# youmi-zym/GO-SLAM

Measured on AMD Instinct MI355X. Metric: BA keyframes/s (6 x FactorGraph.update: reproject + corr lookup + GRU + 2 GN BA iters) on synthetic 640x480 RGB-D, higher is better.
Workload: dtype f32 (BA/geometry; fp64 solve), f16 (corr volume, GRU convs); 1 GPU; configs[1]-shaped frontend window: 60x80 maps (480x640 RGB-D), P=25 keyframes, E=75 edges, 6 updates/keyframe, iters=2, RGB-D depth prior, upsample on; parallelism=replicas x1 (tracking does not shard)

## Files before the change

### go_slam_amd/csrc/gru_gates.hip

```cpp
#include "common.h"

namespace {

typedef _Float16 half8 __attribute__((ext_vector_type(8)));

__device__ __forceinline__ float sigm(float x) { return gs_sigmoid(x); }

__global__ __launch_bounds__(256) void gru_gate_zr_kernel(const _Float16* __restrict__ zr_pre,
                                                          const float* __restrict__ bias,
                                                          const float* __restrict__ glo,
                                                          const _Float16* __restrict__ inp_pre,
                                                          _Float16* __restrict__ hx,
                                                          _Float16* __restrict__ z_out, int hw, int ldx,
                                                          size_t total ) {
  const size_t t = (size_t)blockIdx.x * 256 + threadIdx.x;
  if (t >= total) return;
  const int c8 = (int)(t & 15);
  const size_t pix = t >> 4;
  const int n = (int)(pix / hw);
  const half8 zp = *reinterpret_cast<const half8*>(zr_pre + pix * 256 + c8 * 8);
  const half8 rp = *reinterpret_cast<const half8*>(zr_pre + pix * 256 + 128 + c8 * 8);
  half8* hp = reinterpret_cast<half8*>(hx + pix * ldx + c8 * 8);
  const half8 net = *hp;
  half8 zi = {0, 0, 0, 0, 0, 0, 0, 0}, ri = zi;
  if (inp_pre) {
    zi = *reinterpret_cast<const half8*>(inp_pre + pix * 384 + c8 * 8);
    ri = *reinterpret_cast<const half8*>(inp_pre + pix * 384 + 128 + c8 * 8);
  }
  half8 zo, rn;
#pragma unroll
  for (int k = 0; k < 8; ++k) {
    const int c = c8 * 8 + k;
    const float z = sigm((float)zp[k] + (float)zi[k] + bias[c] + glo[(size_t)n * 256 + c]);
    const float r = sigm((float)rp[k] + (float)ri[k] + bias[128 + c] + glo[(size_t)n * 256 + 128 + c]);
    zo[k] = (_Float16)z;
    rn[k] = (_Float16)(r * (float)net[k]);
  }
  *reinterpret_cast<half8*>(z_out + pix * 128 + c8 * 8) = zo;
  *hp = rn;
}

__global__ __launch_bounds__(256) void gru_gate_q_kernel(const _Float16* __restrict__ q_pre,
                                                         const float* __restrict__ bias,
                                                         const float* __restrict__ glo,
                                                         const _Float16* __restrict__ inp_pre,
                                                         const _Float16* __restrict__ z, const _Float16* __restrict__ net,
                                                         _Float16* __restrict__ net_out, int hw, size_t total) {
  const size_t t = (size_t)blockIdx.x * 256 + threadIdx.x;
  if (t >= total) return;
  const int c8 = (int)(t & 15);
  const size_t pix = t >> 4;
  const int n = (int)(pix / hw);
  const size_t o = pix * 128 + c8 * 8;
  const half8 qp = *reinterpret_cast<const half8*>(q_pre + o);
  const half8 zz = *reinterpret_cast<const half8*>(z + o);
  const half8 nn = *reinterpret_cast<const half8*>(net + o);
  half8 qi = {0, 0, 0, 0, 0, 0, 0, 0};
  if (inp_pre) qi = *reinterpret_cast<const half8*>(inp_pre + pix * 384 + 256 + c8 * 8);
  half8 out;
#pragma unroll
  for (int k = 0; k < 8; ++k) {
    const int c = c8 * 8 + k;
    const float a = (float)qp[k] + (float)qi[k] + bias[c] + glo[(size_t)n * 128 + c];
    const float q = gs_tanh(a);
    const float zf = (float)zz[k];
    out[k] = (_Float16)((1.0f - zf) * (float)nn[k] + zf * q);
  }
  *reinterpret_cast<half8*>(net_out + o) = out;
}

}

extern "C" int gs_gru_gate_zr(const void* zr_pre, const float* bias_zr, const float* glo_zr, const void* inp_pre,
                              void* hx, void* z_out, int n, int hw, int ldx, gs_stream_t stream) {
  GS_REQUIRE(zr_pre && bias_zr && glo_zr && hx && z_out, "gru_gate_zr: null pointer");
  GS_REQUIRE(n >= 0 && hw > 0 && ldx >= 128 && ldx % 8 == 0, "gru_gate_zr: bad shape");
  if (n == 0) return GS_OK;
  const size_t total = (size_t)n * hw * 16;
  gru_gate_zr_kernel<<<(unsigned)((total + 255) / 256), 256, 0, (hipStream_t)stream>>>(
      (const _Float16*)zr_pre, bias_zr, glo_zr, (const _Float16*)inp_pre, (_Float16*)hx, (_Float16*)z_out, hw, ldx,
      total);
  GS_CHECK_LAUNCH("gru_gate_zr");
  return GS_OK;
}

extern "C" int gs_gru_gate_q(const void* q_pre, const float* bias_q, const float* glo_q, const void* inp_pre,
                             const void* z, const void* net, void* net_out, int n, int hw, gs_stream_t stream) {
  GS_REQUIRE(q_pre && bias_q && glo_q && z && net && net_out, "gru_gate_q: null pointer");
  GS_REQUIRE(n >= 0 && hw > 0, "gru_gate_q: bad shape");
  if (n == 0) return GS_OK;
  const size_t total = (size_t)n * hw * 16;
  gru_gate_q_kernel<<<(unsigned)((total + 255) / 256), 256, 0, (hipStream_t)stream>>>(
      (const _Float16*)q_pre, bias_q, glo_q, (const _Float16*)inp_pre, (const _Float16*)z, (const _Float16*)net,
      (_Float16*)net_out, hw, total);
  GS_CHECK_LAUNCH("gru_gate_q");
  return GS_OK;
}

namespace {
template <int ACT, bool BIAS>
__global__ __launch_bounds__(256) void bias_act_kernel(const _Float16* __restrict__ x, const float* __restrict__ bias,
                                                       _Float16* __restrict__ y, int c8n , int ldx, int ldy,
                                                       size_t total ) {
  const size_t t = (size_t)blockIdx.x * 256 + threadIdx.x;
  if (t >= total) return;
  const int c8 = (int)(t % c8n);
  const size_t row = t / c8n;
  half8 v = *reinterpret_cast<const half8*>(x + row * ldx + c8 * 8);
  if (BIAS || ACT) {
#pragma unroll
    for (int k = 0; k < 8; ++k) {
      float f = (float)v[k];
      if (BIAS) f += bias[c8 * 8 + k];
      if (ACT == 1) f = fmaxf(f, 0.0f);
      if (ACT == 2) f = sigm(f);
      v[k] = (_Float16)f;
    }
  }
  *reinterpret_cast<half8*>(y + row * ldy + c8 * 8) = v;
}

__global__ __launch_bounds__(256) void segment_mean_kernel(const _Float16* __restrict__ x, int ldx,
                                                           const float* __restrict__ in_bias, int in_relu,
                                                           const int* __restrict__ off, const int* __restrict__ edges,
                                                           _Float16* __restrict__ out, int hw, int c8n, size_t total) {
  const size_t t = (size_t)blockIdx.x * 256 + threadIdx.x;
  if (t >= total) return;
  const int c8 = (int)(t % c8n);
  const size_t sp = t / c8n;
  const int seg = (int)(sp / hw);
  const int p = (int)(sp - (size_t)seg * hw);
  const int b = off[seg], e = off[seg + 1];
  float bias[8], acc[8];
#pragma unroll
  for (int j = 0; j < 8; ++j) { bias[j] = in_bias ? in_bias[c8 * 8 + j] : 0.0f; acc[j] = 0.0f; }
  const bool touch = (in_bias != nullptr) || in_relu;
  for (int k0 = b; k0 < e; k0 += 4) {
    half8 v[4];
#pragma unroll
    for (int u = 0; u < 4; ++u) {
      const int k = min(k0 + u, e - 1);
      v[u] = *reinterpret_cast<const half8*>(x + ((size_t)edges[k] * hw + p) * ldx + c8 * 8);
    }
#pragma unroll
    for (int u = 0; u < 4; ++u) {
      if (k0 + u >= e) continue;
#pragma unroll
      for (int j = 0; j < 8; ++j) {
        float f = (float)v[u][j];
        if (touch) {
          f += bias[j];
          if (in_relu) f = fmaxf(f, 0.0f);
          f = (float)(_Float16)f;
        }
        acc[j] += f;
      }
    }
  }
  const float inv = e > b ? 1.0f / (float)(e - b) : 0.0f;
  half8 o;
#pragma unroll
  for (int j = 0; j < 8; ++j) o[j] = (_Float16)(acc[j] * inv);
  reinterpret_cast<half8*>(out)[t] = o;
}

__global__ __launch_bounds__(256) void glo_pool_kernel(const _Float16* __restrict__ w_pre, const float* __restrict__ bias,
                                                       const _Float16* __restrict__ net, float* __restrict__ partial,
                                                       int hw, int nchunk) {
  const int n = blockIdx.y, chunk = blockIdx.x;
  const int c8 = threadIdx.x & 15, lane = threadIdx.x >> 4;
  const int p0 = (int)((long)hw * chunk / nchunk), p1 = (int)((long)hw * (chunk + 1) / nchunk);
  float b[8], acc[8];
#pragma unroll
  for (int k = 0; k < 8; ++k) { b[k] = bias[c8 * 8 + k]; acc[k] = 0.0f; }
  for (int p = p0 + lane; p < p1; p += 16) {
    const size_t o = ((size_t)n * hw + p) * 128 + c8 * 8;
    const half8 w = *reinterpret_cast<const half8*>(w_pre + o);
    const half8 h = *reinterpret_cast<const half8*>(net + o);
#pragma unroll
    for (int k = 0; k < 8; ++k) {
      const _Float16 g = (_Float16)sigm((float)(_Float16)((float)w[k] + b[k]));
      acc[k] += (float)(_Float16)((float)g * (float)h[k]);
    }
  }
  __shared__ float red[16][129];
#pragma unroll
  for (int k = 0; k < 8; ++k) red[lane][c8 * 8 + k] = acc[k];
  __syncthreads();
  if (threadIdx.x < 128) {
    float s = 0.0f;
#pragma unroll
    for (int l = 0; l < 16; ++l) s += red[l][threadIdx.x];
    partial[((size_t)n * nchunk + chunk) * 128 + threadIdx.x] = s;
  }
}

typedef _Float16 half4g __attribute__((ext_vector_type(4)));
typedef float float16g __attribute__((ext_vector_type(16)));
__global__ __launch_bounds__(256) void glo_conv_pool_kernel(const _Float16* __restrict__ net, int ldx,
                                                            const _Float16* __restrict__ wpack,
                                                            const float* __restrict__ bias, float* __restrict__ partial,
                                                            int hw, int bpi, size_t nblk) {
  extern __shared__ _Float16 wl[];
  const int tid = threadIdx.x, lane = tid & 63, wv = tid >> 6;
  for (int i = tid; i < 4 * 8 * 64; i += 256) reinterpret_cast<half8*>(wl)[i] = reinterpret_cast<const half8*>(wpack)[i];
  __syncthreads();
  constexpr int TS = 72;
  _Float16* tile = wl + 4 * 8 * 512 + wv * 32 * TS;
  float* sbias = reinterpret_cast<float*>(wl + 4 * 8 * 512 + 4 * 32 * TS);
  if (tid < 128) sbias[tid] = bias[tid];
  __syncthreads();
  const int kh = 8 * (lane >> 5);
  const int piece = lane & 7;
  for (size_t blk = (size_t)blockIdx.x * 4 + wv; blk < nblk; blk += (size_t)gridDim.x * 4) {
    const size_t img = blk / bpi;
    const int b0 = (int)(blk - img * bpi) * 32;
    const int pin = b0 + (lane & 31);
    const _Float16* xr = net + (img * hw + (pin < hw ? pin : hw - 1)) * (size_t)ldx + kh;
    half8 bfr[8];
#pragma unroll
    for (int ks = 0; ks < 8; ++ks) bfr[ks] = *reinterpret_cast<const half8*>(xr + 16 * ks);
    half8 hrow[2][4];
#pragma unroll
    for (int it = 0; it < 4; ++it) {
      const int pxr = b0 + it * 8 + (lane >> 3);
      const _Float16* hr = net + (img * hw + (pxr < hw ? pxr : hw - 1)) * (size_t)ldx + piece * 8;
      hrow[0][it] = *reinterpret_cast<const half8*>(hr);
      hrow[1][it] = *reinterpret_cast<const half8*>(hr + 64);
    }
    float16g c[4];
#pragma unroll
    for (int q = 0; q < 4; ++q)
#pragma unroll
      for (int e = 0; e < 16; ++e) c[q][e] = 0.0f;
#pragma unroll
    for (int ks = 0; ks < 8; ++ks)
#pragma unroll
      for (int q = 0; q < 4; ++q) {
        const half8 a = *reinterpret_cast<const half8*>(wl + ((size_t)(q * 8 + ks) * 64 + lane) * 8);
        c[q] = __builtin_amdgcn_mfma_f32_32x32x16_f16(a, bfr[ks], c[q], 0, 0, 0);
      }
#pragma unroll
    for (int pr = 0; pr < 2; ++pr) {
#pragma unroll
      for (int qq = 0; qq < 2; ++qq)
#pragma unroll
        for (int g = 0; g < 4; ++g) {
          const int chl = qq * 32 + 8 * g + 4 * (lane >> 5);
          half4g o;
#pragma unroll
          for (int e = 0; e < 4; ++e)
            o[e] = (_Float16)sigm((float)(_Float16)(c[2 * pr + qq][4 * g + e] + sbias[pr * 64 + chl + e]));
          *reinterpret_cast<half4g*>(tile + (lane & 31) * TS + chl) = o;
        }
      __builtin_amdgcn_fence(__ATOMIC_RELEASE, "wavefront");
      __builtin_amdgcn_wave_barrier();
      __builtin_amdgcn_fence(__ATOMIC_ACQUIRE, "wavefront");
      float acc[8] = {0.f, 0.f, 0.f, 0.f, 0.f, 0.f, 0.f, 0.f};
#pragma unroll
      for (int it = 0; it < 4; ++it) {
        const int pxr = it * 8 + (lane >> 3);
        const half8 g8 = *reinterpret_cast<const half8*>(tile + pxr * TS + piece * 8);
        const half8 h8 = hrow[pr][it];
        const float live = (b0 + pxr < hw) ? 1.0f : 0.0f;
#pragma unroll
        for (int k = 0; k < 8; ++k) acc[k] += live * (float)(_Float16)((float)g8[k] * (float)h8[k]);
      }
#pragma unroll
      for (int k = 0; k < 8; ++k) {
        acc[k] += __shfl_xor(acc[k], 8);
        acc[k] += __shfl_xor(acc[k], 16);
        acc[k] += __shfl_xor(acc[k], 32);
      }
      if (lane < 8) {
        float* dst = partial + blk * 128 + pr * 64 + lane * 8;
        *reinterpret_cast<float4*>(dst) = make_float4(acc[0], acc[1], acc[2], acc[3]);
        *reinterpret_cast<float4*>(dst + 4) = make_float4(acc[4], acc[5], acc[6], acc[7]);
      }
      __builtin_amdgcn_fence(__ATOMIC_RELEASE, "wavefront");
      __builtin_amdgcn_wave_barrier();
    }
  }
}

__global__ __launch_bounds__(384) void glo_heads_kernel(const float* __restrict__ partial, int nchunk, float inv_hw,
                                                        const _Float16* __restrict__ wz, const _Float16* __restrict__ wr,
                                                        const _Float16* __restrict__ wq, const float* __restrict__ bz,
                                                        const float* __restrict__ br, const float* __restrict__ bq,
                                                        float* __restrict__ gzr, float* __restrict__ gq) {
  const int n = blockIdx.x, t = threadIdx.x;
  __shared__ float g[128];
  __shared__ float part3[3][128];
  {
    const int third = t >> 7, ch = t & 127;
    float s = 0.0f;
    for (int c0 = third; c0 < nchunk; c0 += 30) {
      float v[10];
#pragma unroll
      for (int u = 0; u < 10; ++u) {
        const int c = c0 + 3 * u;
        v[u] = c < nchunk ? partial[((size_t)n * nchunk + c) * 128 + ch] : 0.0f;
      }
#pragma unroll
      for (int u = 0; u < 10; ++u)
        if (c0 + 3 * u < nchunk) s += v[u];
    }
    part3[third][ch] = s;
  }
  __syncthreads();
  if (t < 128) g[t] = (float)(_Float16)(((part3[0][t] + part3[1][t]) + part3[2][t]) * inv_hw);
  __syncthreads();
  const int head = t >> 7, o = t & 127;
  const _Float16* w = (head == 0 ? wz : head == 1 ? wr : wq) + (size_t)o * 128;
  float s = (head == 0 ? bz : head == 1 ? br : bq)[o];
#pragma unroll 4
  for (int k8 = 0; k8 < 16; ++k8) {
    const half8 v = *reinterpret_cast<const half8*>(w + k8 * 8);
#pragma unroll
    for (int k = 0; k < 8; ++k) s = fmaf((float)v[k], g[k8 * 8 + k], s);
  }
  s = (float)(_Float16)s;
  if (head < 2) gzr[(size_t)n * 256 + head * 128 + o] = s;
  else gq[(size_t)n * 128 + o] = s;
}
}

extern "C" int gs_bias_act(const void* x, const float* bias, void* y, int rows, int channels, int x_stride,
                           int y_stride, int act, gs_stream_t stream) {
  GS_REQUIRE(x && y, "bias_act: null pointer");
  GS_REQUIRE(rows >= 0 && channels > 0 && channels % 8 == 0, "bias_act: channels must be a multiple of 8");
  GS_REQUIRE(x_stride >= channels && x_stride % 8 == 0, "bias_act: x_stride must be >= channels and a multiple of 8");
  GS_REQUIRE(y_stride >= channels && y_stride % 8 == 0, "bias_act: y_stride must be >= channels and a multiple of 8");
  GS_REQUIRE(act >= 0 && act <= 2, "bias_act: act in {0 none, 1 relu, 2 sigmoid}");
  if (rows == 0) return GS_OK;
  const size_t total = (size_t)rows * (channels / 8);
  const unsigned grid = (unsigned)((total + 255) / 256);
  hipStream_t st = (hipStream_t)stream;
  const _Float16* xi = (const _Float16*)x;
  _Float16* yo = (_Float16*)y;
  const int c8n = channels / 8;
#define GS_BA(A, B) bias_act_kernel<A, B><<<grid, 256, 0, st>>>(xi, bias, yo, c8n, x_stride, y_stride, total)
  if (bias) { if (act == 0) GS_BA(0, true); else if (act == 1) GS_BA(1, true); else GS_BA(2, true); }
  else      { if (act == 0) GS_BA(0, false); else if (act == 1) GS_BA(1, false); else GS_BA(2, false); }
#undef GS_BA
  GS_CHECK_LAUNCH("bias_act");
  return GS_OK;
}

extern "C" int gs_segment_mean(const void* x, int x_stride, const float* in_bias, int in_relu, const int* seg_offsets,
                               const int* seg_edges, void* out, int n_seg, int hw, int channels, gs_stream_t stream) {
  GS_REQUIRE(x && seg_offsets && seg_edges && out, "segment_mean: null pointer");
  GS_REQUIRE(n_seg >= 0 && hw > 0 && channels > 0 && channels % 8 == 0, "segment_mean: channels must be a multiple of 8");
  GS_REQUIRE(x_stride >= channels && x_stride % 8 == 0, "segment_mean: x_stride must be >= channels, multiple of 8");
  if (n_seg == 0) return GS_OK;
  const size_t total = (size_t)n_seg * hw * (channels / 8);
  segment_mean_kernel<<<(unsigned)((total + 255) / 256), 256, 0, (hipStream_t)stream>>>(
      (const _Float16*)x, x_stride, in_bias, in_relu, seg_offsets, seg_edges, (_Float16*)out, hw, channels / 8, total);
  GS_CHECK_LAUNCH("segment_mean");
  return GS_OK;
}

constexpr int GLO_CHUNKS = 32;
extern "C" size_t gs_gru_glo_workspace_bytes(int n) { return (size_t)(n > 0 ? n : 0) * GLO_CHUNKS * 128 * sizeof(float); }

extern "C" int gs_gru_glo(const void* w_pre, const float* w_bias, const void* net, const void* wz, const void* wr,
                          const void* wq, const float* bz, const float* br, const float* bq, float* gzr, float* gq,
                          int n, int hw, void* workspace, size_t workspace_bytes, gs_stream_t stream) {
  GS_REQUIRE(w_pre && w_bias && net && wz && wr && wq && bz && br && bq && gzr && gq, "gru_glo: null pointer");
  GS_REQUIRE(n >= 0 && hw > 0, "gru_glo: bad shape");
  if (n == 0) return GS_OK;
  GS_REQUIRE(workspace && workspace_bytes >= gs_gru_glo_workspace_bytes(n), "gru_glo: workspace too small");
  hipStream_t st = (hipStream_t)stream;
  const int nchunk = GLO_CHUNKS;
  glo_pool_kernel<<<dim3(nchunk, n), 256, 0, st>>>((const _Float16*)w_pre, w_bias, (const _Float16*)net,
                                                   (float*)workspace, hw, nchunk);
  GS_CHECK_LAUNCH("gru_glo pool");
  glo_heads_kernel<<<n, 384, 0, st>>>((const float*)workspace, nchunk, 1.0f / (float)hw, (const _Float16*)wz,
                                      (const _Float16*)wr, (const _Float16*)wq, bz, br, bq, gzr, gq);
  GS_CHECK_LAUNCH("gru_glo heads");
  return GS_OK;
}

extern "C" size_t gs_gru_glo_fused_workspace_bytes(int n, int hw) {
  if (n <= 0 || hw <= 0) return 0;
  return (size_t)n * ((hw + 31) / 32) * 128 * sizeof(float);
}

extern "C" int gs_gru_glo_fused(const void* net, int net_stride, const void* w_pack, const float* w_bias, const void* wz,
                                const void* wr, const void* wq, const float* bz, const float* br, const float* bq,
                                float* gzr, float* gq, int n, int hw, void* workspace, size_t workspace_bytes,
                                gs_stream_t stream) {
  GS_REQUIRE(net && w_pack && w_bias && wz && wr && wq && bz && br && bq && gzr && gq, "gru_glo_fused: null pointer");
  GS_REQUIRE(n >= 0 && hw > 0 && net_stride >= 128 && net_stride % 8 == 0, "gru_glo_fused: bad shape");
  GS_REQUIRE((((size_t)net | (size_t)w_pack) & 15) == 0, "gru_glo_fused: net / w_pack must be 16-byte aligned");
  if (n == 0) return GS_OK;
  GS_REQUIRE(workspace && workspace_bytes >= gs_gru_glo_fused_workspace_bytes(n, hw), "gru_glo_fused: workspace too small");
  hipStream_t st = (hipStream_t)stream;
  const int bpi = (hw + 31) / 32;
  const size_t nblk = (size_t)n * bpi;
  const size_t lds = (size_t)(4 * 8 * 512 + 4 * 32 * 72) * sizeof(_Float16) + 128 * sizeof(float);
  static GsLdsLimit limit;
  if (int rc = limit.raise((const void*)glo_conv_pool_kernel, lds, "gru_glo_fused")) return rc;
  size_t grid = 256 * 3;
  if (grid > (nblk + 3) / 4) grid = (nblk + 3) / 4;
  glo_conv_pool_kernel<<<(unsigned)grid, 256, lds, st>>>((const _Float16*)net, net_stride, (const _Float16*)w_pack, w_bias,
                                                         (float*)workspace, hw, bpi, nblk);
  GS_CHECK_LAUNCH("gru_glo_fused pool");
  glo_heads_kernel<<<n, 384, 0, st>>>((const float*)workspace, bpi, 1.0f / (float)hw, (const _Float16*)wz,
                                      (const _Float16*)wr, (const _Float16*)wq, bz, br, bq, gzr, gq);
  GS_CHECK_LAUNCH("gru_glo_fused heads");
  return GS_OK;
}

namespace {
__global__ __launch_bounds__(256) void motion_features_kernel(const float2* __restrict__ coords1,
                                                              const float2* __restrict__ target,
                                                              _Float16* __restrict__ out, int hw, int w, size_t total) {
  const size_t t = (size_t)blockIdx.x * 256 + threadIdx.x;
  if (t >= total) return;
  const int p = (int)(t % hw);
  const float gx = (float)(p % w), gy = (float)(p / w);
  const float2 c = coords1[t], tg = target[t];
  typedef _Float16 half4m __attribute__((ext_vector_type(4)));
  half4m o;
  o[0] = (_Float16)gs_clamp_keep_nan(c.x - gx, -64.0f, 64.0f);
  o[1] = (_Float16)gs_clamp_keep_nan(c.y - gy, -64.0f, 64.0f);
  o[2] = (_Float16)gs_clamp_keep_nan(tg.x - c.x, -64.0f, 64.0f);
  o[3] = (_Float16)gs_clamp_keep_nan(tg.y - c.y, -64.0f, 64.0f);
  reinterpret_cast<half4m*>(out)[t] = o;
}

__global__ __launch_bounds__(256) void damping_rows_kernel(const float* __restrict__ eta, const int* __restrict__ inv,
                                                           const int64_t* __restrict__ index,
                                                           float* __restrict__ damping_buf, float* __restrict__ out,
                                                           int hw, float scale, float eps, size_t total) {
  const size_t t = (size_t)blockIdx.x * 256 + threadIdx.x;
  if (t >= total) return;
  const int k = (int)(t / hw), p = (int)(t - (size_t)k * hw);
  const int m = inv[k];
  float* slot = damping_buf + (size_t)index[k] * hw + p;
  float v;
  if (m >= 0) { v = eta[(size_t)m * hw + p]; *slot = v; }
  else v = *slot;
  out[t] = scale * v + eps;
}

__global__ __launch_bounds__(256) void ba_inputs_kernel(const float2* __restrict__ coords1, const float2* __restrict__ delta,
                                                        const float2* __restrict__ weight, float2* __restrict__ target,
                                                        float* __restrict__ ba_target, float* __restrict__ ba_weight,
                                                        int hw, size_t total) {
  const size_t t = (size_t)blockIdx.x * 256 + threadIdx.x;
  if (t >= total) return;
  const size_t e = t / hw;
  const int p = (int)(t - e * hw);
  const float2 c = coords1[t], d = delta[t], wt = weight[t];
  const float2 tg = make_float2(c.x + d.x, c.y + d.y);
  target[t] = tg;
  float* bt = ba_target + e * 2 * hw + p;
  bt[0] = tg.x; bt[hw] = tg.y;
  float* bw = ba_weight + e * 2 * hw + p;
  bw[0] = wt.x; bw[hw] = wt.y;
}
}

extern "C" int gs_motion_features(const float* coords1, const float* target, void* out, int n, int h, int w,
                                  gs_stream_t stream) {
  GS_REQUIRE(coords1 && target && out, "motion_features: null pointer");
  GS_REQUIRE(n >= 0 && h > 0 && w > 0, "motion_features: bad shape");
  if (n == 0) return GS_OK;
  const size_t total = (size_t)n * h * w;
  motion_features_kernel<<<(unsigned)((total + 255) / 256), 256, 0, (hipStream_t)stream>>>(
      (const float2*)coords1, (const float2*)target, (_Float16*)out, h * w, w, total);
  GS_CHECK_LAUNCH("motion_features");
  return GS_OK;
}

extern "C" int gs_ba_inputs(const float* coords1, const float* delta, const float* weight, float* target,
                            float* ba_target, float* ba_weight, int n, int h, int w, gs_stream_t stream) {
  GS_REQUIRE(coords1 && delta && weight && target && ba_target && ba_weight, "ba_inputs: null pointer");
  GS_REQUIRE(n >= 0 && h > 0 && w > 0, "ba_inputs: bad shape");
  if (n == 0) return GS_OK;
  const size_t total = (size_t)n * h * w;
  ba_inputs_kernel<<<(unsigned)((total + 255) / 256), 256, 0, (hipStream_t)stream>>>(
      (const float2*)coords1, (const float2*)delta, (const float2*)weight, (float2*)target, ba_target, ba_weight,
      h * w, total);
  GS_CHECK_LAUNCH("ba_inputs");
  return GS_OK;
}

extern "C" int gs_damping_rows(const float* eta, const int* inv, const int64_t* index, float* damping_buf, float* out,
                               int n_rows, int hw, float scale, float eps, gs_stream_t stream) {
  GS_REQUIRE(inv && index && damping_buf && out, "damping_rows: null pointer");
  GS_REQUIRE(n_rows >= 0 && hw > 0, "damping_rows: bad shape");
  if (n_rows == 0) return GS_OK;
  const size_t total = (size_t)n_rows * hw;
  damping_rows_kernel<<<(unsigned)((total + 255) / 256), 256, 0, (hipStream_t)stream>>>(eta, inv, index, damping_buf, out,
                                                                                       hw, scale, eps, total);
  GS_CHECK_LAUNCH("damping_rows");
  return GS_OK;
}
```

### go_slam_amd/csrc/upsample.hip

```cpp
#include "common.h"

namespace {

__global__ __launch_bounds__(256) void cvx_upsample_kernel(const float* __restrict__ disps,
                                                           const _Float16* __restrict__ mask,
                                                           const int64_t* __restrict__ ix, float* __restrict__ out,
                                                           int m, int h, int w, long cs, long ps) {
  const int lane = threadIdx.x & 63;
  const long pix = (long)blockIdx.x * 4 + (threadIdx.x >> 6);
  const int hw = h * w;
  if (pix >= (long)m * hw) return;
  const int n = (int)(pix / hw), p = (int)(pix - (long)n * hw);
  const int y = p / w, x = p - y * w;
  const long frame = ix ? ix[n] : n;
  const _Float16* mk = mask + (long)n * 576 * hw + (long)p * ps;
  float lg[9], mx = -INFINITY;
#pragma unroll
  for (int k = 0; k < 9; ++k) {
    lg[k] = (float)mk[(long)(k * 64 + lane) * cs];
    mx = fmaxf(mx, lg[k]);
  }
  float den = 0.f;
#pragma unroll
  for (int k = 0; k < 9; ++k) { lg[k] = __expf(lg[k] - mx); den += lg[k]; }
  const float* d = disps + frame * hw;
  const float inv_den = __builtin_amdgcn_rcpf(den);
  float acc = 0.f;
#pragma unroll
  for (int k = 0; k < 9; ++k) {
    const int yy = y + k / 3 - 1, xx = x + k % 3 - 1;
    const float nb = (yy >= 0 && yy < h && xx >= 0 && xx < w) ? d[yy * w + xx] : 0.0f;
    const float wk = (float)(_Float16)(lg[k] * inv_den);
    acc += wk * nb;
  }
  const int i = lane >> 3, j = lane & 7;
  out[frame * (long)hw * 64 + (long)(8 * y + i) * (8 * w) + 8 * x + j] = acc;
}

typedef _Float16 half8u __attribute__((ext_vector_type(8)));
__global__ __launch_bounds__(256) void cvx_upsample_nhwc_kernel(const float* __restrict__ disps,
                                                                const _Float16* __restrict__ mask,
                                                                const int64_t* __restrict__ ix,
                                                                float* __restrict__ out, int m, int h, int w) {
  const int lane = threadIdx.x & 63;
  const long pix = ((long)blockIdx.x * 4 + (threadIdx.x >> 6)) * 8 + (lane >> 3);
  const int hw = h * w;
  if (pix >= (long)m * hw) return;
  const int c = lane & 7;
  const int n = (int)(pix / hw), p = (int)(pix - (long)n * hw);
  const int y = p / w, x = p - y * w;
  const long frame = ix ? ix[n] : n;
  const _Float16* mk = mask + pix * 576 + 8 * c;
  half8u lg[9];
#pragma unroll
  for (int k = 0; k < 9; ++k) lg[k] = *reinterpret_cast<const half8u*>(mk + k * 64);
  const float* d = disps + frame * hw;
  float nb[9];
#pragma unroll
  for (int k = 0; k < 9; ++k) {
    const int yy = y + k / 3 - 1, xx = x + k % 3 - 1;
    nb[k] = (yy >= 0 && yy < h && xx >= 0 && xx < w) ? d[yy * w + xx] : 0.0f;
  }
  float res[8];
#pragma unroll
  for (int j = 0; j < 8; ++j) {
    float e[9], mx = -INFINITY, den = 0.f, acc = 0.f;
#pragma unroll
    for (int k = 0; k < 9; ++k) { e[k] = (float)lg[k][j]; mx = fmaxf(mx, e[k]); }
#pragma unroll
    for (int k = 0; k < 9; ++k) { e[k] = __expf(e[k] - mx); den += e[k]; }
    const float inv_den = __builtin_amdgcn_rcpf(den);
#pragma unroll
    for (int k = 0; k < 9; ++k) acc += (float)(_Float16)(e[k] * inv_den) * nb[k];
    res[j] = acc;
  }
  float4* o = reinterpret_cast<float4*>(out + frame * (long)hw * 64 + (long)(8 * y + c) * (8 * w) + 8 * x);
  o[0] = make_float4(res[0], res[1], res[2], res[3]);
  o[1] = make_float4(res[4], res[5], res[6], res[7]);
}

typedef _Float16 up_h8 __attribute__((ext_vector_type(8)));
typedef float up_f16v __attribute__((ext_vector_type(16)));

__global__ __launch_bounds__(512, 1) void upmask_upsample_kernel(const _Float16* __restrict__ x, int xs,
                                                                 const _Float16* __restrict__ wgt,
                                                                 const float* __restrict__ bias,
                                                                 const float* __restrict__ disps,
                                                                 const int64_t* __restrict__ ix, float* __restrict__ out,
                                                                 int m, int h, int w) {
  const int lane = threadIdx.x & 63, wv = threadIdx.x >> 6;
  const int r = lane & 31, kgl = lane >> 5;
  const int hw = h * w;
  const long total = (long)m * hw;
  up_h8 wa[3][8];
#pragma unroll
  for (int t = 0; t < 3; ++t) {
    const int rowp = 32 * t + r;
    const int ch = (rowp >> 3) * 64 + 8 * wv + (rowp & 7);
#pragma unroll
    for (int s = 0; s < 8; ++s) {
      const up_h8 z = {0, 0, 0, 0, 0, 0, 0, 0};
      wa[t][s] = rowp < 72 ? *reinterpret_cast<const up_h8*>(wgt + (size_t)ch * 128 + 16 * s + 8 * kgl) : z;
    }
  }
  float bv[9][4];
#pragma unroll
  for (int k = 0; k < 9; ++k)
#pragma unroll
    for (int e = 0; e < 4; ++e) bv[k][e] = bias[64 * k + 8 * wv + 4 * kgl + e];
  const long gstride = (long)gridDim.x * 32;
  up_h8 bnext[8];
  long fnext;
  const int64_t* ixp = ix ? ix : reinterpret_cast<const int64_t*>(disps);
  {
    const long g0 = (long)blockIdx.x * 32;
    const long pq0 = (g0 + r < total) ? g0 + r : (g0 < total ? g0 : 0);
    const int n0 = (int)(pq0 / hw);
    { const long f = ixp[n0]; fnext = ix ? f : (long)n0; }
    const _Float16* xr0 = x + (size_t)pq0 * xs + 8 * kgl;
#pragma unroll
    for (int s = 0; s < 8; ++s) bnext[s] = *reinterpret_cast<const up_h8*>(xr0 + 16 * s);
  }
  for (long g0 = (long)blockIdx.x * 32; g0 < total; g0 += gstride) {
    const long pix = g0 + r;
    const bool valid = pix < total;
    const long pq = valid ? pix : g0;
    const int n = (int)(pq / hw), p = (int)(pq - (long)n * hw);
    const long frame = fnext;
    up_h8 bcur[8];
#pragma unroll
    for (int s = 0; s < 8; ++s) bcur[s] = bnext[s];
    {
      const long g1 = g0 + gstride;
      const long pq1 = (g1 + r < total) ? g1 + r : (g1 < total ? g1 : pq);
      const int n1 = (int)(pq1 / hw);
      { const long f = ixp[n1]; fnext = ix ? f : (long)n1; }
      const _Float16* xr1 = x + (size_t)pq1 * xs + 8 * kgl;
#pragma unroll
      for (int s = 0; s < 8; ++s) bnext[s] = *reinterpret_cast<const up_h8*>(xr1 + 16 * s);
    }
    const int y = p / w, xq = p - y * w;
    const float* d = disps + frame * hw;
    float nb[9];
#pragma unroll
    for (int k = 0; k < 9; ++k) {
      const int yy = y + k / 3 - 1, xx = xq + k % 3 - 1;
      const bool in = yy >= 0 && yy < h && xx >= 0 && xx < w;
      const float v = d[min(max(yy, 0), h - 1) * w + min(max(xx, 0), w - 1)];
      nb[k] = in ? v : 0.0f;
    }
    up_f16v acc[3];
#pragma unroll
    for (int t = 0; t < 3; ++t)
#pragma unroll
      for (int e = 0; e < 16; ++e) acc[t][e] = 0.0f;
#pragma unroll
    for (int s = 0; s < 8; ++s) {
#pragma unroll
      for (int t = 0; t < 3; ++t) acc[t] = __builtin_amdgcn_mfma_f32_32x32x16_f16(wa[t][s], bcur[s], acc[t], 0, 0, 0);
    }
    float res[4];
#pragma unroll
    for (int e = 0; e < 4; ++e) {
      float lg[9], mx = -INFINITY, den = 0.f, a = 0.f;
#pragma unroll
      for (int k = 0; k < 9; ++k) {
        lg[k] = (float)(_Float16)(acc[k >> 2][4 * (k & 3) + e] + bv[k][e]);
        mx = fmaxf(mx, lg[k]);
      }
#pragma unroll
      for (int k = 0; k < 9; ++k) { lg[k] = __expf(lg[k] - mx); den += lg[k]; }
      const float inv_den = __builtin_amdgcn_rcpf(den);
#pragma unroll
      for (int k = 0; k < 9; ++k) a += (float)(_Float16)(lg[k] * inv_den) * nb[k];
      res[e] = a;
    }
    if (valid)
      *reinterpret_cast<float4*>(out + frame * (long)hw * 64 + (long)(8 * y + wv) * (8 * w) + 8 * xq + 4 * kgl) =
          make_float4(res[0], res[1], res[2], res[3]);
  }
}

}

extern "C" int gs_cvx_upsample(const float* disps, const void* mask, const int64_t* ix, float* out, int m, int h,
                               int w, int mask_channels_last, gs_stream_t stream) {
  GS_REQUIRE(disps && mask && out, "cvx_upsample: null pointer");
  GS_REQUIRE(m >= 0 && h > 0 && w > 0, "cvx_upsample: bad shape");
  if (m == 0) return GS_OK;
  const long hw = (long)h * w;
  const long cs = mask_channels_last ? 1 : hw, ps = mask_channels_last ? 576 : 1;
  const long total = (long)m * hw;
  if (mask_channels_last) {
    cvx_upsample_nhwc_kernel<<<(unsigned)((total + 31) / 32), 256, 0, (hipStream_t)stream>>>(
        disps, (const _Float16*)mask, ix, out, m, h, w);
    GS_CHECK_LAUNCH("cvx_upsample");
    return GS_OK;
  }
  cvx_upsample_kernel<<<(unsigned)((total + 3) / 4), 256, 0, (hipStream_t)stream>>>(
      disps, (const _Float16*)mask, ix, out, m, h, w, cs, ps);
  GS_CHECK_LAUNCH("cvx_upsample");
  return GS_OK;
}

extern "C" int gs_upmask_upsample(const void* x, int x_stride, const void* weight, const float* bias, const float* disps,
                                  const int64_t* ix, float* out, int m, int h, int w, gs_stream_t stream) {
  GS_REQUIRE(x && weight && bias && disps && out, "upmask_upsample: null pointer");
  GS_REQUIRE(m >= 0 && h > 0 && w > 0 && x_stride >= 128 && x_stride % 8 == 0, "upmask_upsample: bad shape");
  GS_REQUIRE((8 * w) % 4 == 0, "upmask_upsample: bad width");
  if (m == 0) return GS_OK;
  const long total = (long)m * h * w;
  long blocks = (total + 31) / 32;
  if (blocks > 256) blocks = 256;
  upmask_upsample_kernel<<<(unsigned)blocks, 512, 0, (hipStream_t)stream>>>(
      (const _Float16*)x, x_stride, (const _Float16*)weight, bias, disps, ix, out, m, h, w);
  GS_CHECK_LAUNCH("upmask_upsample");
  return GS_OK;
}
```

Measured before the change: 85.33 keyframes/s.

## Stage upmask input rows through LDS double buffer and reindex segment_mean grid

segment_mean now launches a 2D grid with one y-block per segment and a power-of-two channel lane split. This removes 64-bit divides and hoists the pixel base pointer. The upmask upsample kernel now stages each 32-pixel group's 128-channel rows cooperatively into a double-buffered shared-memory tile, with coalesced loads and one prefetch in flight, instead of per-lane register prefetch of strided rows. It also caches frame indices in dynamic LDS, uses 32-bit index math, and tweaks the rounding of the softmax weight product using inline asm. It adds a __syncthreads per iteration and new shape limits.

```diff
diff --git a/go_slam_amd/csrc/gru_gates.hip b/go_slam_amd/csrc/gru_gates.hip
--- a/go_slam_amd/csrc/gru_gates.hip
+++ b/go_slam_amd/csrc/gru_gates.hip
@@ -123,24 +123,23 @@
 __global__ __launch_bounds__(256) void segment_mean_kernel(const _Float16* __restrict__ x, int ldx,
                                                            const float* __restrict__ in_bias, int in_relu,
                                                            const int* __restrict__ off, const int* __restrict__ edges,
-                                                           _Float16* __restrict__ out, int hw, int c8n, size_t total) {
-  const size_t t = (size_t)blockIdx.x * 256 + threadIdx.x;
-  if (t >= total) return;
-  const int c8 = (int)(t % c8n);
-  const size_t sp = t / c8n;
-  const int seg = (int)(sp / hw);
-  const int p = (int)(sp - (size_t)seg * hw);
+                                                           _Float16* __restrict__ out, int hw, int c8n, int cshift) {
+  const int seg = blockIdx.y;
+  const int c8 = threadIdx.x & ((1 << cshift) - 1);
+  const int p = (int)((blockIdx.x * 256u + threadIdx.x) >> cshift);
+  if (p >= hw || c8 >= c8n) return;
   const int b = off[seg], e = off[seg + 1];
   float bias[8], acc[8];
 #pragma unroll
   for (int j = 0; j < 8; ++j) { bias[j] = in_bias ? in_bias[c8 * 8 + j] : 0.0f; acc[j] = 0.0f; }
   const bool touch = (in_bias != nullptr) || in_relu;
+  const _Float16* xp = x + (size_t)p * ldx + c8 * 8;
   for (int k0 = b; k0 < e; k0 += 4) {
     half8 v[4];
 #pragma unroll
     for (int u = 0; u < 4; ++u) {
       const int k = min(k0 + u, e - 1);
-      v[u] = *reinterpret_cast<const half8*>(x + ((size_t)edges[k] * hw + p) * ldx + c8 * 8);
+      v[u] = *reinterpret_cast<const half8*>(xp + (size_t)edges[k] * hw * ldx);
     }
 #pragma unroll
     for (int u = 0; u < 4; ++u) {
@@ -161,7 +160,7 @@
   half8 o;
 #pragma unroll
   for (int j = 0; j < 8; ++j) o[j] = (_Float16)(acc[j] * inv);
-  reinterpret_cast<half8*>(out)[t] = o;
+  reinterpret_cast<half8*>(out)[((size_t)seg * hw + p) * c8n + c8] = o;
 }
 
 __global__ __launch_bounds__(256) void glo_pool_kernel(const _Float16* __restrict__ w_pre, const float* __restrict__ bias,
@@ -353,9 +352,13 @@
   GS_REQUIRE(n_seg >= 0 && hw > 0 && channels > 0 && channels % 8 == 0, "segment_mean: channels must be a multiple of 8");
   GS_REQUIRE(x_stride >= channels && x_stride % 8 == 0, "segment_mean: x_stride must be >= channels, multiple of 8");
   if (n_seg == 0) return GS_OK;
-  const size_t total = (size_t)n_seg * hw * (channels / 8);
-  segment_mean_kernel<<<(unsigned)((total + 255) / 256), 256, 0, (hipStream_t)stream>>>(
-      (const _Float16*)x, x_stride, in_bias, in_relu, seg_offsets, seg_edges, (_Float16*)out, hw, channels / 8, total);
+  GS_REQUIRE(n_seg <= 65535 && channels <= 2048 && hw <= (1 << 23), "segment_mean: shape out of range");
+  const int c8n = channels / 8;
+  int cshift = 0;
+  while ((1 << cshift) < c8n) ++cshift;
+  const unsigned per_block = 256u >> cshift;
+  segment_mean_kernel<<<dim3(((unsigned)hw + per_block - 1) / per_block, (unsigned)n_seg), 256, 0, (hipStream_t)stream>>>(
+      (const _Float16*)x, x_stride, in_bias, in_relu, seg_offsets, seg_edges, (_Float16*)out, hw, c8n, cshift);
   GS_CHECK_LAUNCH("segment_mean");
   return GS_OK;
 }
diff --git a/go_slam_amd/csrc/upsample.hip b/go_slam_amd/csrc/upsample.hip
--- a/go_slam_amd/csrc/upsample.hip
+++ b/go_slam_amd/csrc/upsample.hip
@@ -81,6 +81,13 @@
 
 typedef _Float16 up_h8 __attribute__((ext_vector_type(8)));
 typedef float up_f16v __attribute__((ext_vector_type(16)));
+__device__ __forceinline__ _Float16 up_mul_round_once(float a, float b) {
+  unsigned r;
+  asm("v_fma_mixlo_f16 %0, %1, %2, 0" : "=v"(r) : "v"(a), "v"(b));
+  return __builtin_bit_cast(_Float16, (unsigned short)(r & 0xffffu));
+}
+constexpr int UP_TS = 136;
+constexpr int UP_MAX_FRAMES = 8192;
 
 __global__ __launch_bounds__(512, 1) void upmask_upsample_kernel(const _Float16* __restrict__ x, int xs,
                                                                  const _Float16* __restrict__ wgt,
@@ -88,10 +95,14 @@
                                                                  const float* __restrict__ disps,
                                                                  const int64_t* __restrict__ ix, float* __restrict__ out,
                                                                  int m, int h, int w) {
-  const int lane = threadIdx.x & 63, wv = threadIdx.x >> 6;
+  __shared__ __attribute__((aligned(16))) _Float16 rows[2][32 * UP_TS];
+  extern __shared__ int frames[];
+  const int tid = threadIdx.x, lane = tid & 63, wv = tid >> 6;
   const int r = lane & 31, kgl = lane >> 5;
-  const int hw = h * w;
-  const long total = (long)m * hw;
+  const unsigned hw = (unsigned)(h * w);
+  const unsigned total = (unsigned)m * hw;
+  if (ix)
+    for (int i = tid; i < m; i += 512) frames[i] = (int)ix[i];
   up_h8 wa[3][8];
 #pragma unroll
   for (int t = 0; t < 3; ++t) {
@@ -108,47 +119,36 @@
   for (int k = 0; k < 9; ++k)
 #pragma unroll
     for (int e = 0; e < 4; ++e) bv[k][e] = bias[64 * k + 8 * wv + 4 * kgl + e];
-  const long gstride = (long)gridDim.x * 32;
-  up_h8 bnext[8];
-  long fnext;
-  const int64_t* ixp = ix ? ix : reinterpret_cast<const int64_t*>(disps);
-  {
-    const long g0 = (long)blockIdx.x * 32;
-    const long pq0 = (g0 + r < total) ? g0 + r : (g0 < total ? g0 : 0);
-    const int n0 = (int)(pq0 / hw);
-    { const long f = ixp[n0]; fnext = ix ? f : (long)n0; }
-    const _Float16* xr0 = x + (size_t)pq0 * xs + 8 * kgl;
-#pragma unroll
-    for (int s = 0; s < 8; ++s) bnext[s] = *reinterpret_cast<const up_h8*>(xr0 + 16 * s);
-  }
-  for (long g0 = (long)blockIdx.x * 32; g0 < total; g0 += gstride) {
-    const long pix = g0 + r;
+  const unsigned gstride = gridDim.x * 32u;
+  const unsigned sp = (unsigned)tid >> 4, sc = (unsigned)tid & 15;
+  const _Float16* xcol = x + 8 * sc;
+  const unsigned soff = sp * UP_TS + 8 * sc;
+  unsigned g0 = blockIdx.x * 32u;
+  *reinterpret_cast<up_h8*>(&rows[0][soff]) =
+      *reinterpret_cast<const up_h8*>(xcol + (size_t)min(g0 + sp, total - 1) * xs);
+  up_h8 stage = *reinterpret_cast<const up_h8*>(xcol + (size_t)min(g0 + gstride + sp, total - 1) * xs);
+  const unsigned foff = r * UP_TS + 8 * kgl;
+  for (int cur = 0; g0 < total; g0 += gstride, cur ^= 1) {
+    __syncthreads();
+    const unsigned pix = g0 + r;
     const bool valid = pix < total;
-    const long pq = valid ? pix : g0;
-    const int n = (int)(pq / hw), p = (int)(pq - (long)n * hw);
-    const long frame = fnext;
-    up_h8 bcur[8];
-#pragma unroll
-    for (int s = 0; s < 8; ++s) bcur[s] = bnext[s];
-    {
-      const long g1 = g0 + gstride;
-      const long pq1 = (g1 + r < total) ? g1 + r : (g1 < total ? g1 : pq);
-      const int n1 = (int)(pq1 / hw);
-      { const long f = ixp[n1]; fnext = ix ? f : (long)n1; }
-      const _Float16* xr1 = x + (size_t)pq1 * xs + 8 * kgl;
-#pragma unroll
-      for (int s = 0; s < 8; ++s) bnext[s] = *reinterpret_cast<const up_h8*>(xr1 + 16 * s);
-    }
-    const int y = p / w, xq = p - y * w;
-    const float* d = disps + frame * hw;
-    float nb[9];
+    const unsigned pq = valid ? pix : g0;
+    const unsigned n = pq / hw, p = pq - n * hw;
+    const long frame = ix ? (long)frames[n] : (long)n;
+    const int y = (int)(p / (unsigned)w), xq = (int)p - y * w;
+    const float* d = disps + frame * (long)hw;
+    float nbv[9];
+    bool nbin[9];
 #pragma unroll
     for (int k = 0; k < 9; ++k) {
       const int yy = y + k / 3 - 1, xx = xq + k % 3 - 1;
-      const bool in = yy >= 0 && yy < h && xx >= 0 && xx < w;
-      const float v = d[min(max(yy, 0), h - 1) * w + min(max(xx, 0), w - 1)];
-      nb[k] = in ? v : 0.0f;
-    }
+      nbin[k] = yy >= 0 && yy < h && xx >= 0 && xx < w;
+      nbv[k] = d[min(max(yy, 0), h - 1) * w + min(max(xx, 0), w - 1)];
+    }
+    up_h8 bcur[8];
+#pragma unroll
+    for (int s = 0; s < 8; ++s) bcur[s] = *reinterpret_cast<const up_h8*>(&rows[cur][foff + 16 * s]);
+    __builtin_amdgcn_sched_barrier(0);
     up_f16v acc[3];
 #pragma unroll
     for (int t = 0; t < 3; ++t)
@@ -159,6 +159,9 @@
 #pragma unroll
       for (int t = 0; t < 3; ++t) acc[t] = __builtin_amdgcn_mfma_f32_32x32x16_f16(wa[t][s], bcur[s], acc[t], 0, 0, 0);
     }
+    float nb[9];
+#pragma unroll
+    for (int k = 0; k < 9; ++k) nb[k] = nbin[k] ? nbv[k] : 0.0f;
     float res[4];
 #pragma unroll
     for (int e = 0; e < 4; ++e) {
@@ -172,12 +175,25 @@
       for (int k = 0; k < 9; ++k) { lg[k] = __expf(lg[k] - mx); den += lg[k]; }
       const float inv_den = __builtin_amdgcn_rcpf(den);
 #pragma unroll
-      for (int k = 0; k < 9; ++k) a += (float)(_Float16)(lg[k] * inv_den) * nb[k];
+      for (int k = 0; k < 9; ++k) {
+        _Float16 wk;
+        if (k == 0) {
+          wk = up_mul_round_once(inv_den, lg[k]);
+        } else {
+          float pk = lg[k] * inv_den;
+          asm("" : "+v"(pk));
+          wk = (_Float16)pk;
+        }
+        a += (float)wk * nb[k];
+      }
       res[e] = a;
     }
+    asm volatile("" : "+v"(res[0]), "+v"(res[1]), "+v"(res[2]), "+v"(res[3]));
     if (valid)
       *reinterpret_cast<float4*>(out + frame * (long)hw * 64 + (long)(8 * y + wv) * (8 * w) + 8 * xq + 4 * kgl) =
           make_float4(res[0], res[1], res[2], res[3]);
+    *reinterpret_cast<up_h8*>(&rows[cur ^ 1][soff]) = stage;
+    stage = *reinterpret_cast<const up_h8*>(xcol + (size_t)min(g0 + 2 * gstride + sp, total - 1) * xs);
   }
 }
 
@@ -210,9 +226,11 @@
   GS_REQUIRE((8 * w) % 4 == 0, "upmask_upsample: bad width");
   if (m == 0) return GS_OK;
   const long total = (long)m * h * w;
+  GS_REQUIRE(total <= 0x7fff0000L && (long)h * w <= 0x7fffffffL, "upmask_upsample: m * h * w must fit in 32 bits");
+  GS_REQUIRE(!ix || m <= UP_MAX_FRAMES, "upmask_upsample: at most 8192 indexed frames per call");
   long blocks = (total + 31) / 32;
   if (blocks > 256) blocks = 256;
-  upmask_upsample_kernel<<<(unsigned)blocks, 512, 0, (hipStream_t)stream>>>(
+  upmask_upsample_kernel<<<(unsigned)blocks, 512, ix ? (size_t)m * sizeof(int) : 0, (hipStream_t)stream>>>(
       (const _Float16*)x, x_stride, (const _Float16*)weight, bias, disps, ix, out, m, h, w);
   GS_CHECK_LAUNCH("upmask_upsample");
   return GS_OK;
```

Measured after the change: 86.03 keyframes/s (median of 6 runs). About the same (+0.8%).
